# Mahdi-Si/VAE-TEB

Measured on AMD Instinct MI355X. Metric: train samples/sec + ELBO, 4096-pt windows, batch 256, 1/2/4/8 MI355X, higher is better.
Workload: dtype bf16 MFMA (decoder heads + conv blocks + ResidualMLP linears, LSTM recurrences f16 fwd / bf16 bwd), fp32 accumulation; fp32 LayerNorm / BatchNorm / LSTM state / front-end / optimizer

## Files before the change

include/vaeteb.h:

```cpp
#ifndef VAETEB_H
#define VAETEB_H

#include <stdint.h>

#ifdef __cplusplus
extern "C" {
#endif

#define VT_OK 0
#define VT_ERR_ARG (-1)
#define VT_ERR_LAYOUT (-2)
#define VT_ERR_HIP (-3)

#define VT_FFT_MAX_LDS 8192

const char* vt_last_error(void);
int vt_stream_fork(void* from, void* to);
int vt_stream_mark(void* stream, int* slot);
int vt_stream_wait_mark(void* stream, int slot);
int vt_abi_version(void);
int vt_arrive_reset(void* stream);
int vt_capture_info(void* stream, char* buf, int len);
int vt_set_h16_format(int fp16);
int vt_get_h16_format(void);


int vt_fe_spectrum(const float* x, int64_t rows, int N, int n_pad, int pad_left, int pad_mode, const void* tw,
                   void* xhat, void* stream);
int vt_fe_spectrum_rolled(const float* x, int64_t B, int64_t x_row_stride, int N, int n_pad, int pad_left,
                          int pad_mode, const int* shifts, int K, const void* tw, void* xhat, void* stream);

int vt_fe_lowpass(const float* x, int64_t rows, int64_t x_row_stride, int N, int n_pad, int pad_left,
                  const float* h0, int radius, int step, int start, int S, float* out, int64_t out_row_stride,
                  void* stream);

int vt_fe_wavelet(const void* xhat, int64_t B, int C, int n_pad, const float* psi, int n_items, const int* items,
                  const void* tw, int N, int pad_left, void* analytic, int n_slots, const float* h0, int radius,
                  int step, int start, int S, float* s1, int s1_channels, void* stream);

int vt_fe_pairs(const void* analytic, int64_t B, int n_slots, int N, int n_pad, int pad_left, int n_pairs,
                const int* slot_i, const int* slot_j, const float* power, const void* tw, const float* phi0, int dec,
                int start, int S, int pad_mode, float* out, void* stream);
int vt_fe_pairs_split(const void* analytic_i, int n_slots_i, const void* analytic_j, int n_slots_j, int64_t B, int K,
                      int N, int n_pad, int pad_left, int n_pairs, const int* slot_i, const int* slot_j,
                      const float* power, const void* tw, const float* phi0, int dec, int start, int S,
                      int pad_mode, float* out, void* stream);

int vt_fe_set_pairs_persist(int grid);
int vt_fe_set_pairs_direct(int on);
int vt_fe_set_pairs_half(int on);
int vt_fe_set_analytic_polar(int on);

int vt_fe_set_pairs_stamps(void* buf);

int vt_fe_normalize(const float* in, int64_t B, int C, int in_C, int S, const int* kind, const float* mean, const float* stdv,
                    float log_eps, float* out, int out_C, int out_off, void* stream);
int vt_fe_normalize_window(const float* in, int64_t B, int C, int in_C, int in_S, int s0, int S_len,
// ... 348 lines not shown
```

vae-teb_amd/csrc/abi.cpp:

```cpp
#include <stdarg.h>
#include <stdio.h>
#include <stdlib.h>

#include <atomic>
#include <utility>
#include <vector>

#include "common.h"

namespace vt {
static thread_local char g_err[512] = "";

void set_error(const char* fmt, ...) {
    va_list ap;
    va_start(ap, fmt);
    vsnprintf(g_err, sizeof(g_err), fmt, ap);
    va_end(ap);
}

unsigned arrive_slots(unsigned n, hipStream_t st) {
    static std::atomic<unsigned> next[2];
    constexpr unsigned HALF = ARRIVE_POOL / 2;
    hipStreamCaptureStatus cs = hipStreamCaptureStatusNone;
    const int cap = (st && hipStreamIsCapturing(st, &cs) == hipSuccess && cs == hipStreamCaptureStatusActive) ? 1 : 0;
    for (;;) {
        const unsigned b = next[cap].fetch_add(n) % HALF;
        if (b + n <= HALF) return b + cap * HALF;
    }
}

static std::vector<std::pair<const void*, size_t>>& arrive_pools() {
    static std::vector<std::pair<const void*, size_t>> v;
    return v;
}
int register_arrive_pool(const void* sym, size_t bytes) {
    arrive_pools().emplace_back(sym, bytes);
    return (int)arrive_pools().size();
}

static std::atomic<int> g_h16{0};
int h16_format() { return g_h16.load(std::memory_order_relaxed); }
}

extern "C" {
const char* vt_last_error(void) { return vt::g_err; }

int vt_arrive_reset(void* stream) {
    for (const auto& [sym, bytes] : vt::arrive_pools()) {
        void* p = nullptr;
        if (hipGetSymbolAddress(&p, sym) != hipSuccess || hipMemsetAsync(p, 0, bytes, vt::S(stream)) != hipSuccess) {
            vt::set_error("vt_arrive_reset: cannot clear a counter pool");
            return VT_ERR_HIP;
        }
    }
    return VT_OK;
}
int vt_abi_version(void) { return 1; }
int vt_set_h16_format(int fp16) { return vt::g_h16.exchange(fp16 ? 1 : 0); }
int vt_get_h16_format(void) { return vt::h16_format(); }
}

namespace {
constexpr int kForkEvents = 1024, kMaxDevices = 16;
hipEvent_t g_fork_ev[kMaxDevices][kForkEvents];
std::atomic<unsigned> g_fork_next[kMaxDevices];

struct SlotRec {
    unsigned long long cap;
    void* stream;
};
SlotRec g_slot[kMaxDevices][kForkEvents];
int g_trace = -1;

unsigned long long capture_id(void* stream, bool* capturing) {
    hipStreamCaptureStatus st = hipStreamCaptureStatusNone;
    unsigned long long id = 0;
    if (hipStreamGetCaptureInfo((hipStream_t)stream, &st, &id) != hipSuccess) {
        (void)hipGetLastError();
        st = hipStreamCaptureStatusNone;
    }
    *capturing = st == hipStreamCaptureStatusActive;
    return *capturing ? id : 0ull;
}

bool trace() {
    if (g_trace < 0) {
        const char* e = getenv("VAETEB_EVENT_TRACE");
        g_trace = e && e[0] == '1';
    }
    return g_trace;
}
}
// ... 118 lines not shown
```

vae-teb_amd/csrc/common.h:

```cpp
#pragma once
#include <hip/hip_runtime.h>
#include <stdint.h>

#include "../../include/vaeteb.h"

namespace vt {

void set_error(const char* fmt, ...);
const void* bucket_marker_kernel();

#define VT_CHECK_ARG(cond, ...)                  \
    do {                                         \
        if (!(cond)) {                           \
            ::vt::set_error(__VA_ARGS__);        \
            return VT_ERR_ARG;                   \
        }                                        \
    } while (0)

#define VT_LAUNCH_CHECK(name)                                                     \
    do {                                                                          \
        hipError_t e_ = hipGetLastError();                                        \
        if (e_ != hipSuccess) {                                                   \
            ::vt::set_error("%s: %s", name, hipGetErrorString(e_));               \
            return VT_ERR_HIP;                                                    \
// ... 40 lines not shown
}

__device__ __forceinline__ bool last_arrival(unsigned* ctr, unsigned total) {
    __shared__ unsigned s_last;
    asm volatile("s_waitcnt vmcnt(0)" ::: "memory");
    __syncthreads();
    if (threadIdx.x == 0) {
        const unsigned old = atomicAdd(ctr, 1u);
        const bool last = old == total - 1;
        if (last) atomicExch(ctr, 0u);
        s_last = last ? 1u : 0u;
    }
    __syncthreads();
    return s_last != 0u;
}

__device__ __forceinline__ float wave_sum(float v) {
#pragma unroll
    for (int o = 32; o > 0; o >>= 1) v += __shfl_xor(v, o, 64);
    return v;
}

__device__ __forceinline__ float block_sum(float v, float* red) {
    v = wave_sum(v);
    const int lane = threadIdx.x & 63, w = threadIdx.x >> 6, nw = (blockDim.x + 63) >> 6;
    __syncthreads();
    if (lane == 0) red[w] = v;
    __syncthreads();
    float t = 0.f;
    for (int i = 0; i < nw; ++i) t += red[i];
    return t;
}

__device__ __forceinline__ int reflect_idx(int i, int n) {
    if (n == 1) return 0;
    const int p = 2 * (n - 1);
    i %= p;
    if (i < 0) i += p;
    return i < n ? i : p - i;
}

__device__ __forceinline__ int pad_src(int i, int n, int mode) {
    if (mode == 0) return reflect_idx(i, n);
    if (mode == 1) return (i < 0 || i >= n) ? -1 : i;
    i %= n;
    return i < 0 ? i + n : i;
}

}
```

vae-teb_amd/csrc/gemm.hip:

```cpp
#include <algorithm>

#include "common.h"
#include "skinny.h"

namespace vt {

static constexpr int TM = 64, TN = 64, TK = 16, GT = 256;

struct RowMajor {
    const float* p;
    int64_t ld;
    __device__ float at(int64_t r, int64_t c) const { return p[r * ld + c]; }
};
struct ColMajor {
    const float* p;
    int64_t ld;
    __device__ float at(int64_t r, int64_t c) const { return p[c * ld + r]; }
};

struct ConvGeom {
    int B, L_in, Cin, Cout, K;
    int up;
    int mode;
    int L_up;
// ... 176 lines not shown
            for (; r + 3 * rpi < r1; r += 4 * rpi) {
                a0 += X[r * N + c];
                a1 += X[(r + rpi) * N + c];
                a2 += X[(r + 2 * rpi) * N + c];
                a3 += X[(r + 3 * rpi) * N + c];
            }
            for (; r < r1; r += rpi) a0 += X[r * N + c];
        }
        const float a = (a0 + a1) + (a2 + a3);
        red[threadIdx.x] = a;
        __syncthreads();
        if (threadIdx.x < N) {
            float s = 0.f;
            for (int i = 0; i < rpi; ++i) s += red[i * N + threadIdx.x];
            partial[(int64_t)blockIdx.x * N + threadIdx.x] = s;
        }
    } else {
        const int n = blockIdx.y * 256 + threadIdx.x;
        if (n >= N) return;
        float a = 0.f;
        for (int64_t r = r0; r < r1; ++r) a += X[r * N + n];
        partial[(int64_t)blockIdx.x * N + n] = a;
    }
}
__global__ __launch_bounds__(256) void k_colsum_final(const float* __restrict__ partial, int blocks, int N,
                                                      float* __restrict__ out, int accumulate) {
    __shared__ float red[16];
    const int n = blockIdx.x;
    float a = 0.f;
#pragma unroll 8
    for (int b = threadIdx.x; b < blocks; b += 256) a += partial[(int64_t)b * N + n];
    a = block_sum(a, red);
    if (threadIdx.x == 0) out[n] = accumulate ? out[n] + a : a;
}

template <bool UP>
__global__ void k_conv_fold(const float* __restrict__ gpad, ConvGeom g, float rcin, float* __restrict__ dx,
                            int accumulate) {
    const int i = blockIdx.x * blockDim.x + threadIdx.x;
    if (i >= g.L_in * g.Cin) return;
    const int b = blockIdx.y;
    const int Lp = g.L_out + g.K - 1;
    const float* gb0 = gpad + (int64_t)b * Lp * g.Cin;
    float out;
    if (!UP && g.mode == 0) {
        out = gb0[g.pad * g.Cin + i];
    } else {
        int s = rcin != 0.f ? (int)((float)i * rcin) : i / g.Cin;
        if (s * g.Cin > i) --s;
        else if ((s + 1) * g.Cin <= i) ++s;
        const int ci = i - s * g.Cin;
        const float* gb = gb0 + ci;
        auto gup = [&](int t) -> float {
            float v = gb[(t + g.pad) * g.Cin];
            if (g.mode == 0) return v;
            if (g.L_up <= g.pad) {
                if (t == 0)
                    for (int tp = 0; tp < g.pad; ++tp) v += gb[tp * g.Cin];
                if (t == g.L_up - 1)
                    for (int tp = g.pad + g.L_up; tp < Lp; ++tp) v += gb[tp * g.Cin];
                return v;
            }
            if (t >= 1 && t <= g.pad) v += gb[(g.pad - t) * g.Cin];
            const int tr = g.pad + 2 * (g.L_up - 1) - t;
            if (t <= g.L_up - 2 && tr < Lp && tr >= g.pad + g.L_up) v += gb[tr * g.Cin];
            return v;
// ... 127 lines not shown
                                                  K, nullptr, accumulate, ws, ws_floats, vt_gemm_splits_hint(N, K, R),
                                                  0, 0, 0, S(stream));
}

int vt_conv1d_fold(const float* gpad, int B, int L_in, int Cin, int Cout, int K, int mode, int up, float* dX,
                   int accumulate, void* stream) {
    VT_CHECK_ARG(B > 0 && L_in > 0 && Cin > 0, "vt_conv1d_fold: shape");
    ConvGeom g = make_geom(B, L_in, Cin, Cout, K, mode, up);
    const int rc = fold_launch(gpad, g, dX, accumulate, S(stream));
    if (rc) return rc;
    VT_LAUNCH_CHECK("vt_conv1d_fold");
    return VT_OK;
}

int vt_linear_ln_fwd(const float* X, int64_t R, int K, const float* W, int N, const float* bias, const float* gamma,
                     const float* beta, int act, float eps, float* Y, float* xhat, float* rstd, void* stream) {
    VT_CHECK_ARG(R > 0 && K > 0 && N > 0 && N <= SK_MAX_N && gamma && beta && act >= 0 && act <= 3,
                 "vt_linear_ln_fwd: shape (N <= %d)", SK_MAX_N);
    sk_linear_ln_fwd(X, R, K, W, N, bias, gamma, beta, act, eps, Y, xhat, rstd, S(stream));
    VT_LAUNCH_CHECK("vt_linear_ln_fwd");
    return VT_OK;
}

int vt_colsum(const float* X, int64_t R, int N, float* out, int accumulate, float* ws, int64_t ws_floats,
              void* stream) {
    VT_CHECK_ARG(R > 0 && N > 0, "vt_colsum: shape");
    const int64_t rows = N <= 256 ? 64 : 8;
    int64_t blocks = (R + rows - 1) / rows;
    if (blocks > 1024) blocks = 1024;
    if (blocks * N > ws_floats) blocks = ws_floats / N;
    VT_CHECK_ARG(blocks >= 1, "vt_colsum: workspace too small");
    const int64_t rpb = (R + blocks - 1) / blocks;
    blocks = (R + rpb - 1) / rpb;
    hipLaunchKernelGGL(k_colsum_partial, dim3((unsigned)blocks, N <= 256 ? 1 : (unsigned)((N + 255) / 256)),
                       dim3(256), 0, S(stream), X, R, N, rpb, ws);
    hipLaunchKernelGGL(k_colsum_final, dim3(N), dim3(256), 0, S(stream), ws, (int)blocks, N, out,
                       accumulate);
    VT_LAUNCH_CHECK("vt_colsum");
    return VT_OK;
}

int vt_conv1d_out_len(int L_in, int K, int mode, int up) { return make_geom(1, L_in, 1, 1, K, mode, up).L_out; }

int vt_conv1d_fwd(const float* X, int B, int L_in, int Cin, const float* W, int Cout, int K, int mode, int up,
                  float* Y, void* stream) {
    VT_CHECK_ARG(B > 0 && L_in > 0 && Cin > 0 && Cout > 0 && K > 0 && (mode == 0 || mode == 1),
                 "vt_conv1d_fwd: shape");
    ConvGeom g = make_geom(B, L_in, Cin, Cout, K, mode, up);
    VT_CHECK_ARG(mode == 0 || g.L_up > 1, "vt_conv1d_fwd: length");
    const int64_t M = (int64_t)B * g.L_out;
    return launch<Im2col, ConvW, false, false>("vt_conv1d_fwd", Im2col{X, g}, ConvW{W, Cin, K}, M, Cout,
                                               (int64_t)K * Cin, Y, Cout, nullptr, 0, nullptr, 0, 1, 0, 0, 0,
                                               S(stream));
}

int vt_conv1d_bwd_data(const float* dY, int B, int L_in, int Cin, const float* W, int Cout, int K, int mode, int up,
                       float* dX, int accumulate, float* gpad, void* stream) {
    VT_CHECK_ARG(B > 0 && L_in > 0 && Cin > 0 && Cout > 0 && K > 0, "vt_conv1d_bwd_data: shape");
    ConvGeom g = make_geom(B, L_in, Cin, Cout, K, mode, up);
    const int Lp = g.L_out + K - 1;
    const int64_t M = (int64_t)B * Lp;
    int rc = launch<Col2imA, ConvWT, false, false>("vt_conv1d_bwd_data", Col2imA{dY, g.L_out, Lp, Cout},
                                                   ConvWT{W, Cin, Cout, K}, M, Cin, (int64_t)K * Cout, gpad, Cin,
                                                   nullptr, 0, nullptr, 0, 1, 0, 0, 0, S(stream));
    if (rc) return rc;
    rc = fold_launch(gpad, g, dX, accumulate, S(stream));
// ... 19 lines not shown
```

vae-teb_amd/csrc/mfma.hip:

```cpp
#include "h16.h"

namespace vt {

constexpr int QM = 256, QN = 64, QK = 64, QT = 512;
constexpr int ROWB = QK * 2;
constexpr int A_BYTES = QM * ROWB;
constexpr int B_BYTES = QN * ROWB;
constexpr int NA = 3, NB = 8;
constexpr int GEMM_LDS = NA * A_BYTES + NB * B_BYTES;

__device__ __forceinline__ int swz(int r, int c) { return c ^ ((r >> 1) & 7); }

__device__ __forceinline__ void glds16(const void* src, char* lds) {
    __builtin_amdgcn_global_load_lds((const __attribute__((address_space(1))) void*)src,
                                     (__attribute__((address_space(3))) void*)lds, 16, 0, 0);
}

VT_ARRIVE_POOL(g_arrive_gemm);

typedef unsigned u32x4 __attribute__((ext_vector_type(4)));
__device__ __forceinline__ void st_agent4(__amdgpu_buffer_rsrc_t r, unsigned off, f32x4 v) {
    __builtin_amdgcn_raw_buffer_store_b128(__builtin_bit_cast(u32x4, v), r, (int)off, 0, CPOL_SC1);
}
__device__ __forceinline__ f32x4 ld_agent4(__amdgpu_buffer_rsrc_t r, unsigned off) {
// ... 106 lines not shown
                s += p == z ? acc[g >> 2][g & 3] : ld_agent4(pr, (unsigned)(p * slab + (g * QT + tid) * 16));
            acc[g >> 2][g & 3] = s;
        }
    }
#pragma unroll
    for (int i = 0; i < 2; ++i)
#pragma unroll
        for (int j = 0; j < 4; ++j) {
            const int col = n0 + 16 * j + lr;
            const float bcol = bias ? bias[col] : 0.f;
#pragma unroll
            for (int r = 0; r < 4; ++r) {
                const int row = m0 + 32 * w + 16 * i + 4 * lc + r;
                if (row >= M) continue;
                float o = acc[i][j][r] + bcol;
                if (accumulate) o = C[(int64_t)row * ldc + col] + o;
                C[(int64_t)row * ldc + col] = o;
            }
        }
}

template <typename H>
__global__ void k_bf16_rows(const float* __restrict__ X, int64_t M, int K, H* __restrict__ out, int64_t Mpad,
                            int Kpad) {
    const int64_t i = (int64_t)blockIdx.x * blockDim.x + threadIdx.x;
    const int64_t total = Mpad * Kpad;
    if (i >= total) return;
    const int64_t m = i / Kpad;
    const int k = (int)(i - m * Kpad);
    out[i] = (m < M && k < K) ? (H)X[m * K + k] : (H)0.f;
}

template <typename H>
__global__ __launch_bounds__(256) void k_bf16_transpose(const float* __restrict__ X, int64_t R, int Cn,
                                                        H* __restrict__ out, int64_t Cpad, int64_t Rpad) {
    __shared__ float tile[64][65];
    const int64_t r0 = (int64_t)blockIdx.x * 64, c0 = (int64_t)blockIdx.y * 64;
    const int tx = threadIdx.x & 63, ty = threadIdx.x >> 6;
    for (int i = ty; i < 64; i += 4) {
        const int64_t r = r0 + i, c = c0 + tx;
        tile[i][tx] = (r < R && c < Cn) ? X[r * Cn + c] : 0.f;
    }
    __syncthreads();
    for (int i = ty; i < 64; i += 4) {
        const int64_t c = c0 + i, r = r0 + tx;
        if (c < Cpad && r < Rpad) out[c * Rpad + r] = (H)tile[tx][i];
    }
}

template <typename H>
__global__ __launch_bounds__(256) void k_bf16_shadow(const float* __restrict__ W, int N, int K,
                                                     H* __restrict__ W16, H* __restrict__ W16t) {
    __shared__ float tile[64][65];
    const int64_t n0 = (int64_t)blockIdx.y * 64, k0 = (int64_t)blockIdx.x * 64;
    const int tx = threadIdx.x & 63, ty = threadIdx.x >> 6;
    for (int i = ty; i < 64; i += 4) {
        const float v = W[(n0 + i) * K + k0 + tx];
        tile[i][tx] = v;
        W16[(n0 + i) * K + k0 + tx] = (H)v;
    }
    __syncthreads();
    for (int i = ty; i < 64; i += 4) W16t[(k0 + i) * N + n0 + tx] = (H)tile[tx][i];
}

typedef short v4i16 __attribute__((ext_vector_type(4)));
typedef short v8i16 __attribute__((ext_vector_type(8)));
// ... 136 lines not shown

}

using namespace vt;

extern "C" {

int vt_mfma_supported(int K, int N) { return (K > 0 && N > 0 && K % QK == 0 && N % QN == 0) ? 1 : 0; }

int vt_mfma_workspace_floats(int64_t R, int K, int N, int64_t* floats) {
    VT_CHECK_ARG(R > 0 && K > 0 && N > 0 && floats, "vt_mfma_workspace_floats: shape");
    MfmaPlan f = plan(R, N, K), d = plan(R, K, N), w = plan(N, K, R);
    const int64_t wf = w.a_floats + up_to((int64_t)K * w.Kpad / 2, 64) + w.part_floats + N;
    int64_t m = f.a_floats + f.part_floats;
    if (d.a_floats + d.part_floats > m) m = d.a_floats + d.part_floats;
    if (wf > m) m = wf;
    *floats = m;
    return VT_OK;
}

int vt_mfma_weight_shadow(const float* W, int N, int K, void* W16, void* W16t, void* stream) {
    VT_CHECK_ARG(vt_mfma_supported(K, N) && W && W16 && W16t, "vt_mfma_weight_shadow: K and N must be multiples of 64");
    VT_H16(hipLaunchKernelGGL(k_bf16_shadow<H>, dim3(K / 64, N / 64), dim3(256), 0, S(stream), W, N, K, (H*)W16,
                              (H*)W16t));
    VT_LAUNCH_CHECK("vt_mfma_weight_shadow");
    return VT_OK;
}

int vt_mfma_linear_fwd(const float* X, int64_t R, int K, const void* W16, int N, const float* bias, float* Y,
                       float* ws, int64_t ws_floats, void* stream) {
    VT_CHECK_ARG(R > 0 && vt_mfma_supported(K, N), "vt_mfma_linear_fwd: K and N must be positive multiples of 64");
    MfmaPlan p = plan(R, N, K);
    VT_CHECK_ARG(p.a_floats + p.part_floats <= ws_floats, "vt_mfma_linear_fwd: workspace too small");
    const int64_t tot = p.Mpad * p.Kpad;
    int rc = VT_OK;
    VT_H16(H* A = (H*)ws;
           hipLaunchKernelGGL(k_bf16_rows<H>, dim3((unsigned)((tot + 255) / 256)), dim3(256), 0, S(stream), X, R, K, A,
                              p.Mpad, (int)p.Kpad);
           rc = run("vt_mfma_linear_fwd", (const H*)A, (const H*)W16, K, R, N, p, Y, bias, 0, ws + p.a_floats,
                    S(stream)));
    return rc;
}

int vt_mfma_linear_bwd_data(const float* dY, int64_t R, int N, const void* W16t, int K, float* dX, int accumulate,
                            float* ws, int64_t ws_floats, void* stream) {
    VT_CHECK_ARG(R > 0 && vt_mfma_supported(N, K), "vt_mfma_linear_bwd_data: K and N must be positive multiples of 64");
    MfmaPlan p = plan(R, K, N);
    VT_CHECK_ARG(p.a_floats + p.part_floats <= ws_floats, "vt_mfma_linear_bwd_data: workspace too small");
    const int64_t tot = p.Mpad * p.Kpad;
    int rc = VT_OK;
    VT_H16(H* A = (H*)ws;
           hipLaunchKernelGGL(k_bf16_rows<H>, dim3((unsigned)((tot + 255) / 256)), dim3(256), 0, S(stream), dY, R, N, A,
                              p.Mpad, (int)p.Kpad);
           rc = run("vt_mfma_linear_bwd_data", (const H*)A, (const H*)W16t, N, R, K, p, dX, nullptr, accumulate,
                    ws + p.a_floats, S(stream)));
    return rc;
}

int vt_mfma_linear_bwd_weight(const float* dY, int64_t R, int N, const float* X, int K, float* dW, float* db,
                              int accumulate, float* ws, int64_t ws_floats, void* stream) {
    VT_CHECK_ARG(R > 0 && vt_mfma_supported(K, N), "vt_mfma_linear_bwd_weight: K and N must be positive multiples of 64");
    if (N % DWT == 0 && K % DWT == 0) {
        VT_H16(hipLaunchKernelGGL(k_mfma_dw<H>, dim3(K / DWT, N / DWT), dim3(256), 0, S(stream), dY, R, N, X, K, dW,
                                  accumulate));
        VT_LAUNCH_CHECK("vt_mfma_linear_bwd_weight");
        return db ? vt_colsum(dY, R, N, db, accumulate, ws, ws_floats, stream) : VT_OK;
    }
    MfmaPlan p = plan(N, K, R);
    const int64_t b_floats = up_to((int64_t)K * p.Kpad / 2, 64);
    VT_CHECK_ARG(p.a_floats + b_floats + p.part_floats + N <= ws_floats, "vt_mfma_linear_bwd_weight: workspace too small");
    float* part = ws + p.a_floats + b_floats;
    int rc = VT_OK;
    VT_H16(H* A = (H*)ws;
           H* Bt = (H*)(ws + p.a_floats);
           hipLaunchKernelGGL(k_bf16_transpose<H>, dim3((unsigned)(p.Kpad / 64), (unsigned)(p.Mpad / 64)), dim3(256), 0,
                              S(stream), dY, R, N, A, p.Mpad, p.Kpad);
           hipLaunchKernelGGL(k_bf16_transpose<H>, dim3((unsigned)(p.Kpad / 64), (unsigned)(K / 64)), dim3(256), 0,
                              S(stream), X, R, K, Bt, (int64_t)K, p.Kpad);
           rc = run("vt_mfma_linear_bwd_weight", (const H*)A, (const H*)Bt, p.Kpad, N, K, p, dW, nullptr, accumulate,
                    part, S(stream)));
    if (rc || !db) return rc;
    return vt_colsum(dY, R, N, db, accumulate, part, ws_floats - p.a_floats - b_floats, stream);
}

}
```

vae-teb_amd/csrc/norm.hip:

```cpp
#include <math.h>
#include <stdlib.h>

#include "bnbwd.h"
#include "common.h"
#include "dropout.h"

namespace vt {

enum Act { ACT_NONE = 0, ACT_RELU = 1, ACT_GELU = 2, ACT_TANH = 3 };

__device__ __forceinline__ float act_f(float z, int act) {
    switch (act) {
        case ACT_RELU: return z > 0.f ? z : 0.f;
        case ACT_GELU: return 0.5f * z * (1.f + erff(z * 0.70710678118654752f));
        case ACT_TANH: return tanhf(z);
        default: return z;
    }
}
__device__ __forceinline__ float act_d(float z, int act) {
    switch (act) {
        case ACT_RELU: return z > 0.f ? 1.f : 0.f;
        case ACT_GELU: {
            const float cdf = 0.5f * (1.f + erff(z * 0.70710678118654752f));
            const float pdf = 0.39894228040143268f * expf(-0.5f * z * z);
// ... 139 lines not shown
            b += red[i][1][c];
        }
        part[(int64_t)blockIdx.x * 2 * C + c] = a;
        part[(int64_t)blockIdx.x * 2 * C + C + c] = b;
    }
}

__global__ __launch_bounds__(NT) void k_ln_bwd_wide(const float* __restrict__ dy, const float* __restrict__ xhat,
                                                    const float* __restrict__ rstd, int C,
                                                    const float* __restrict__ gamma, const float* __restrict__ beta,
                                                    int act, float* __restrict__ dx, float* __restrict__ rowpart) {
    __shared__ float red[16];
    const int64_t row = blockIdx.x;
    const float* dyr = dy + row * C;
    const float* hr = xhat + row * C;
    float s1 = 0.f, s2 = 0.f;
    for (int c = threadIdx.x; c < C; c += NT) {
        const float h = hr[c];
        const float dz = dyr[c] * act_d(h * gamma[c] + beta[c], act);
        const float g = dz * gamma[c];
        s1 += g;
        s2 += g * h;
        rowpart[row * 2 * C + c] = dz * h;
        rowpart[row * 2 * C + C + c] = dz;
    }
    const float m1 = block_sum(s1, red) / (float)C;
    const float m2 = block_sum(s2, red) / (float)C;
    const float rs = rstd[row];
    for (int c = threadIdx.x; c < C; c += NT) {
        const float h = hr[c];
        const float dz = dyr[c] * act_d(h * gamma[c] + beta[c], act);
        dx[row * C + c] = rs * (dz * gamma[c] - m1 - h * m2);
    }
}

template <int CTRL>
__device__ __forceinline__ float dppf(float v) {
    return __builtin_bit_cast(float, __builtin_amdgcn_update_dpp(0, __builtin_bit_cast(int, v), CTRL, 0xF, 0xF, false));
}
__device__ __forceinline__ float sum16(float v) {
    v += dppf<0xB1>(v);
    v += dppf<0x4E>(v);
    const float r4 = dppf<0x124>(v), r12 = dppf<0x12C>(v);
    v += (threadIdx.x & 4) ? r4 : r12;
    v += dppf<0x128>(v);
    return v;
}

template <int CPL>
__global__ __launch_bounds__(NT) void k_ln_fwd16(const float* __restrict__ x, int64_t R, int C,
                                                 const float* __restrict__ gamma, const float* __restrict__ beta,
                                                 int act, float eps, float* __restrict__ y, float* __restrict__ xhat,
                                                 float* __restrict__ rstd_out) {
    const int lr = threadIdx.x & 15;
    const int64_t row = (int64_t)blockIdx.x * (NT / 16) + (threadIdx.x >> 4);
    const bool ok = row < R;
    const float* xr = x + (ok ? row : 0) * C;
    float v[CPL], s = 0.f;
#pragma unroll
    for (int j = 0; j < CPL; ++j) {
        const int c = lr + 16 * j;
        v[j] = (ok && c < C) ? xr[c] : 0.f;
        s += v[j];
    }
    const float mean = sum16(s) / (float)C;
    float q = 0.f;
// ... 809 lines not shown
                     float* ws, int64_t ws_floats, void* stream) {
    VT_CHECK_ARG(R > 0 && C > 0, "vt_layernorm_bwd: shape");
    hipStream_t st = S(stream);
    if (C <= 256) {
        int64_t blocks = (R + 63) / 64;
        if (blocks > 1024) blocks = 1024;
        if (blocks * 2 * C > ws_floats) blocks = ws_floats / (2 * C);
        VT_CHECK_ARG(blocks >= 1, "vt_layernorm_bwd: workspace too small");
        const int64_t rpb = (R + blocks - 1) / blocks;
        blocks = (R + rpb - 1) / rpb;
        const dim3 grid((unsigned)blocks);
#define VT_LNB(CPL) hipLaunchKernelGGL(k_ln_bwd16<CPL>, grid, dim3(NT), 0, st, dy, xhat, rstd, R, C, gamma, beta, act, \
                                       rpb, dx, ws)
        if (C <= 32) VT_LNB(2);
        else if (C <= 64) VT_LNB(4);
        else if (C <= 128) VT_LNB(8);
        else VT_LNB(16);
#undef VT_LNB
        hipLaunchKernelGGL(k_colred16, dim3((unsigned)((2 * C + CR_C - 1) / CR_C)), dim3(NT), 0, st, ws, (int)blocks,
                           2 * C, dgamma, dbeta, C, accumulate_params);
    } else if (C <= 512) {
        int64_t blocks = (R + 63) / 64;
        if (blocks > 1024) blocks = 1024;
        if (blocks * 2 * C > ws_floats) blocks = ws_floats / (2 * C);
        VT_CHECK_ARG(blocks >= 1, "vt_layernorm_bwd: workspace too small");
        const int64_t rpb = (R + blocks - 1) / blocks;
        blocks = (R + rpb - 1) / rpb;
        hipLaunchKernelGGL(k_ln_bwd<8>, dim3((unsigned)blocks), dim3(NT), 0, st, dy, xhat, rstd, R, C, gamma, beta,
                           act, rpb, dx, ws);
        hipLaunchKernelGGL(k_reduce_parts, dim3(2 * C), dim3(NT), 0, st, ws, (int)blocks, 2 * C, dgamma,
                           dbeta, C, accumulate_params);
    } else {
        VT_CHECK_ARG(ws_floats >= 2 * R * C, "vt_layernorm_bwd: workspace too small (wide)");
        hipLaunchKernelGGL(k_ln_bwd_wide, dim3((unsigned)R), dim3(NT), 0, st, dy, xhat, rstd, C, gamma, beta, act, dx,
                           ws);
        hipLaunchKernelGGL(k_reduce_parts, dim3(2 * C), dim3(NT), 0, st, ws, (int)R, 2 * C, dgamma, dbeta,
                           C, accumulate_params);
    }
    VT_LAUNCH_CHECK("vt_layernorm_bwd");
    return VT_OK;
}

static int bn_blocks(int64_t M, int64_t ws_floats, int C, int64_t* rpb) {
    auto need = [&](int64_t b) { return ((2 * C * b + 1) & ~(int64_t)1) + 4 * C * ((b + BN_GB - 1) / BN_GB); };
    int64_t blocks = (M + 255) / 256;
    const int64_t cap = C <= 128 && g_bn_fold ? BN_FOLD_BLOCKS : 2048;
    if (blocks > cap) blocks = cap;
    while (blocks > 1 && need(blocks) > ws_floats) blocks = blocks * 15 / 16 < blocks - 1 ? blocks * 15 / 16 : blocks - 1;
    if (need(blocks) > ws_floats) return 0;
    *rpb = ((M + blocks - 1) / blocks + 3) / 4 * 4;
    return (int)((M + *rpb - 1) / *rpb);
}

static BnFin fin_of(int mode, int64_t M) {
    BnFin f{};
    f.mode = mode;
    f.M = M;
    return f;
}

int vt_batchnorm_fwd(const float* x, int64_t M, int C, const float* gamma, const float* beta, int act, float eps,
                     float momentum, float* y, float* mean, float* rstd, float* run_mean, float* run_var, float* ws,
                     int64_t ws_floats, void* stream) {
    VT_CHECK_ARG(M > 0 && C > 0 && C <= 256, "vt_batchnorm_fwd: shape (C <= 256)");
    int64_t rpb;
    const int blocks = bn_blocks(M, ws_floats, C, &rpb);
    VT_CHECK_ARG(blocks >= 1, "vt_batchnorm_fwd: workspace too small");
    hipStream_t st = S(stream);
    BnFin f0 = fin_of(0, M);
    f0.mean = mean;
// ... 200 lines not shown
```

vae-teb_amd/vaeteb/_lib.py:

```python
import ctypes
import os
import re

import torch

_HERE = os.path.dirname(os.path.abspath(__file__))
_ROOT = os.path.dirname(os.path.dirname(_HERE))
LIB_PATH = os.environ.get("VAETEB_LIB", os.path.join(_HERE, "_lib", "libvaeteb.so"))
HEADER = os.path.join(_ROOT, "include", "vaeteb.h")

VT_ERR_ARG, VT_ERR_LAYOUT, VT_ERR_HIP = -1, -2, -3

_CT = {
    "int": ctypes.c_int, "int64_t": ctypes.c_int64, "float": ctypes.c_float, "double": ctypes.c_double,
    "void*": ctypes.c_void_p, "float*": ctypes.c_void_p, "double*": ctypes.c_void_p, "int*": ctypes.c_void_p, "int32_t*": ctypes.c_void_p, "int64_t*": ctypes.c_void_p,
    "char*": ctypes.c_char_p,
}


def parse_header(path=HEADER):
    src = open(path).read()
    src = re.sub(r"/\*.*?\*/", " ", src, flags=re.S)
    protos = {}
    for m in re.finditer(r"\b(const\s+char\s*\*|int|void)\s+(vt_\w+)\s*\(([^)]*)\)\s*;", src):
# ... 70 lines not shown


def stream():
    return torch._C._cuda_getCurrentRawStream(torch._C._cuda_getDevice())


def call(name, *args):
    return lib().call(name, *args)


def wait_for(waiter, src=None):
    w = waiter if isinstance(waiter, int) else waiter.cuda_stream
    s = stream() if src is None else (src if isinstance(src, int) else src.cuda_stream)
    if w != s:
        rc = lib().fns["vt_stream_fork"](s, w)
        if rc != 0:
            raise RuntimeError(f"vt_stream_fork: {lib().last_error()}")


_H16 = [None]


def set_h16(fp16):
    v = 1 if fp16 else 0
    if _H16[0] != v:
        lib().fns["vt_set_h16_format"](v)
        _H16[0] = v


def h16():
    return "fp16" if lib().fns["vt_get_h16_format"]() else "bf16"


def capture_info(src=None):
    import ctypes
    buf = ctypes.create_string_buffer(1 << 16)
    s = stream() if src is None else (src if isinstance(src, int) else src.cuda_stream)
    call("vt_capture_info", s, buf, len(buf))
    return buf.value.decode()


def mark(src=None):
    import ctypes
    slot = ctypes.c_int()
    call("vt_stream_mark", stream() if src is None else src.cuda_stream, ctypes.byref(slot))
    return slot.value


def wait_mark(slot, waiter=None):
    call("vt_stream_wait_mark", stream() if waiter is None else waiter.cuda_stream, slot)
```

Baseline: 34070.

## Fuse wide LayerNorm backward and column sums into single-pass kernels; vectorize bf16 row packing

```diff
diff --git a/include/vaeteb.h b/include/vaeteb.h
--- a/include/vaeteb.h
+++ b/include/vaeteb.h
@@ -23,6 +23,7 @@
 int vt_capture_info(void* stream, char* buf, int len);
 int vt_set_h16_format(int fp16);
 int vt_get_h16_format(void);
+int vt_set_wide_glue_legacy(int on);
 
 
 int vt_fe_spectrum(const float* x, int64_t rows, int N, int n_pad, int pad_left, int pad_mode, const void* tw,
diff --git a/vae-teb_amd/csrc/abi.cpp b/vae-teb_amd/csrc/abi.cpp
--- a/vae-teb_amd/csrc/abi.cpp
+++ b/vae-teb_amd/csrc/abi.cpp
@@ -40,6 +40,9 @@
 
 static std::atomic<int> g_h16{0};
 int h16_format() { return g_h16.load(std::memory_order_relaxed); }
+
+static std::atomic<int> g_wide_legacy{getenv("VAETEB_WIDE_GLUE_LEGACY") ? atoi(getenv("VAETEB_WIDE_GLUE_LEGACY")) != 0 : 0};
+int wide_glue_legacy() { return g_wide_legacy.load(std::memory_order_relaxed); }
 }
 
 extern "C" {
@@ -58,6 +61,7 @@
 int vt_abi_version(void) { return 1; }
 int vt_set_h16_format(int fp16) { return vt::g_h16.exchange(fp16 ? 1 : 0); }
 int vt_get_h16_format(void) { return vt::h16_format(); }
+int vt_set_wide_glue_legacy(int on) { return vt::g_wide_legacy.exchange(on ? 1 : 0); }
 }
 
 namespace {
diff --git a/vae-teb_amd/csrc/common.h b/vae-teb_amd/csrc/common.h
--- a/vae-teb_amd/csrc/common.h
+++ b/vae-teb_amd/csrc/common.h
@@ -96,6 +96,32 @@
     return t;
 }
 
+constexpr int CT_C = 16;
+__device__ __forceinline__ void ct_wave_sums(float (&a)[CT_C], float (*red)[CT_C]) {
+    const int lane = threadIdx.x & 63, w = threadIdx.x >> 6;
+#pragma unroll
+    for (int o = 32; o > 0; o >>= 1) {
+        float t[CT_C];
+#pragma unroll
+        for (int j = 0; j < CT_C; ++j) t[j] = __shfl_xor(a[j], o, 64);
+#pragma unroll
+        for (int j = 0; j < CT_C; ++j) a[j] += t[j];
+    }
+    if (lane == 0) {
+#pragma unroll
+        for (int j = 0; j < CT_C; ++j) red[w][j] = a[j];
+    }
+    __syncthreads();
+}
+__device__ __forceinline__ float ct_total(const float (*red)[CT_C], int j) {
+    float t = 0.f;
+#pragma unroll
+    for (int i = 0; i < 4; ++i) t += red[i][j];
+    return t;
+}
+
+int wide_glue_legacy();
+
 __device__ __forceinline__ int reflect_idx(int i, int n) {
     if (n == 1) return 0;
     const int p = 2 * (n - 1);
diff --git a/vae-teb_amd/csrc/gemm.hip b/vae-teb_amd/csrc/gemm.hip
--- a/vae-teb_amd/csrc/gemm.hip
+++ b/vae-teb_amd/csrc/gemm.hip
@@ -232,6 +232,55 @@
     for (int b = threadIdx.x; b < blocks; b += 256) a += partial[(int64_t)b * N + n];
     a = block_sum(a, red);
     if (threadIdx.x == 0) out[n] = accumulate ? out[n] + a : a;
+}
+
+__global__ __launch_bounds__(256) void k_colsum_wide(const float* __restrict__ X, int64_t M, int N,
+                                                     int64_t rows_per_block, int blocks, float* __restrict__ out,
+                                                     int accumulate) {
+    static_assert(CT_C == 16, "16 columns x 16 partial groups");
+    __shared__ float sp[256][CT_C + 1];
+    __shared__ float red[4][CT_C];
+    const int tid = threadIdx.x, cc = tid & (CT_C - 1), q = tid >> 4;
+    const int c0 = blockIdx.x * CT_C, c = c0 + cc;
+    float acc[CT_C];
+#pragma unroll
+    for (int j = 0; j < CT_C; ++j) acc[j] = 0.f;
+    for (int b0 = 0; b0 < blocks; b0 += 256) {
+        for (int i = 0; i < 16; i += 2) {
+            const int ba = b0 + q + 16 * i, bb = ba + 16;
+            if (ba >= blocks) break;
+            const int64_t r0a = (int64_t)ba * rows_per_block, r0b = (int64_t)bb * rows_per_block;
+            const int64_t r1a = c >= N ? r0a : (r0a + rows_per_block < M ? r0a + rows_per_block : M);
+            const int64_t r1b = c >= N || bb >= blocks ? r0b : (r0b + rows_per_block < M ? r0b + rows_per_block : M);
+            float pa = 0.f, pb = 0.f;
+            for (int64_t k = 0; k < rows_per_block; k += 8) {
+                float va[8], vb[8];
+#pragma unroll
+                for (int u = 0; u < 8; ++u) {
+                    va[u] = r0a + k + u < r1a ? X[(r0a + k + u) * N + c] : 0.f;
+                    vb[u] = r0b + k + u < r1b ? X[(r0b + k + u) * N + c] : 0.f;
+                }
+#pragma unroll
+                for (int u = 0; u < 8; ++u) {
+                    if (r0a + k + u < r1a) pa += va[u];
+                    if (r0b + k + u < r1b) pb += vb[u];
+                }
+            }
+            sp[q + 16 * i][cc] = pa;
+            if (bb < blocks) sp[q + 16 * i + 16][cc] = pb;
+        }
+        __syncthreads();
+        if (b0 + tid < blocks) {
+#pragma unroll
+            for (int j = 0; j < CT_C; ++j) acc[j] += sp[tid][j];
+        }
+        __syncthreads();
+    }
+    ct_wave_sums(acc, red);
+    if (tid < CT_C && c0 + tid < N) {
+        const float v = ct_total(red, tid);
+        out[c0 + tid] = accumulate ? out[c0 + tid] + v : v;
+    }
 }
 
 template <bool UP>
@@ -425,6 +474,12 @@
     VT_CHECK_ARG(blocks >= 1, "vt_colsum: workspace too small");
     const int64_t rpb = (R + blocks - 1) / blocks;
     blocks = (R + rpb - 1) / rpb;
+    if (N > 256 && R <= 16384 && !wide_glue_legacy()) {
+        hipLaunchKernelGGL(k_colsum_wide, dim3((unsigned)((N + CT_C - 1) / CT_C)), dim3(256), 0, S(stream), X, R, N, rpb,
+                           (int)blocks, out, accumulate);
+        VT_LAUNCH_CHECK("vt_colsum");
+        return VT_OK;
+    }
     hipLaunchKernelGGL(k_colsum_partial, dim3((unsigned)blocks, N <= 256 ? 1 : (unsigned)((N + 255) / 256)),
                        dim3(256), 0, S(stream), X, R, N, rpb, ws);
     hipLaunchKernelGGL(k_colsum_final, dim3(N), dim3(256), 0, S(stream), ws, (int)blocks, N, out,
diff --git a/vae-teb_amd/csrc/mfma.hip b/vae-teb_amd/csrc/mfma.hip
--- a/vae-teb_amd/csrc/mfma.hip
+++ b/vae-teb_amd/csrc/mfma.hip
@@ -162,6 +162,33 @@
 }
 
 template <typename H>
+__global__ __launch_bounds__(256) void k_bf16_rows4(const float4* __restrict__ X, int64_t M, int K4,
+                                                    hv4<H>* __restrict__ out, int64_t Mpad, int Kpad4) {
+    const int k4 = blockIdx.x * 64 + (threadIdx.x & 63);
+    if (k4 >= Kpad4) return;
+    for (int64_t m = (int64_t)blockIdx.y * 4 + (threadIdx.x >> 6); m < Mpad; m += 4 * (int64_t)gridDim.y) {
+        hv4<H> o = {(H)0.f, (H)0.f, (H)0.f, (H)0.f};
+        if (m < M && k4 < K4) {
+            const float4 v = X[m * K4 + k4];
+            o = hv4<H>{(H)v.x, (H)v.y, (H)v.z, (H)v.w};
+        }
+        out[m * Kpad4 + k4] = o;
+    }
+}
+
+template <typename H>
+static void launch_rows(const float* X, int64_t M, int K, H* out, int64_t Mpad, int Kpad, hipStream_t st) {
+    if (K % 4 == 0 && Kpad % 4 == 0 && (uintptr_t)X % 16 == 0 && (uintptr_t)out % 8 == 0 && !wide_glue_legacy()) {
+        const int64_t gy = (Mpad + 3) / 4;
+        hipLaunchKernelGGL(k_bf16_rows4<H>, dim3((unsigned)((Kpad / 4 + 63) / 64), (unsigned)(gy < 65535 ? gy : 65535)),
+                           dim3(256), 0, st, (const float4*)X, M, K / 4, (hv4<H>*)out, Mpad, Kpad / 4);
+        return;
+    }
+    const int64_t tot = Mpad * Kpad;
+    hipLaunchKernelGGL(k_bf16_rows<H>, dim3((unsigned)((tot + 255) / 256)), dim3(256), 0, st, X, M, K, out, Mpad, Kpad);
+}
+
+template <typename H>
 __global__ __launch_bounds__(256) void k_bf16_transpose(const float* __restrict__ X, int64_t R, int Cn,
                                                         H* __restrict__ out, int64_t Cpad, int64_t Rpad) {
     __shared__ float tile[64][65];
@@ -364,11 +391,9 @@
     VT_CHECK_ARG(R > 0 && vt_mfma_supported(K, N), "vt_mfma_linear_fwd: K and N must be positive multiples of 64");
     MfmaPlan p = plan(R, N, K);
     VT_CHECK_ARG(p.a_floats + p.part_floats <= ws_floats, "vt_mfma_linear_fwd: workspace too small");
-    const int64_t tot = p.Mpad * p.Kpad;
     int rc = VT_OK;
     VT_H16(H* A = (H*)ws;
-           hipLaunchKernelGGL(k_bf16_rows<H>, dim3((unsigned)((tot + 255) / 256)), dim3(256), 0, S(stream), X, R, K, A,
-                              p.Mpad, (int)p.Kpad);
+           launch_rows<H>(X, R, K, A, p.Mpad, (int)p.Kpad, S(stream));
            rc = run("vt_mfma_linear_fwd", (const H*)A, (const H*)W16, K, R, N, p, Y, bias, 0, ws + p.a_floats,
                     S(stream)));
     return rc;
@@ -379,11 +404,9 @@
     VT_CHECK_ARG(R > 0 && vt_mfma_supported(N, K), "vt_mfma_linear_bwd_data: K and N must be positive multiples of 64");
     MfmaPlan p = plan(R, K, N);
     VT_CHECK_ARG(p.a_floats + p.part_floats <= ws_floats, "vt_mfma_linear_bwd_data: workspace too small");
-    const int64_t tot = p.Mpad * p.Kpad;
     int rc = VT_OK;
     VT_H16(H* A = (H*)ws;
-           hipLaunchKernelGGL(k_bf16_rows<H>, dim3((unsigned)((tot + 255) / 256)), dim3(256), 0, S(stream), dY, R, N, A,
-                              p.Mpad, (int)p.Kpad);
+           launch_rows<H>(dY, R, N, A, p.Mpad, (int)p.Kpad, S(stream));
            rc = run("vt_mfma_linear_bwd_data", (const H*)A, (const H*)W16t, N, R, K, p, dX, nullptr, accumulate,
                     ws + p.a_floats, S(stream)));
     return rc;
diff --git a/vae-teb_amd/csrc/norm.hip b/vae-teb_amd/csrc/norm.hip
--- a/vae-teb_amd/csrc/norm.hip
+++ b/vae-teb_amd/csrc/norm.hip
@@ -195,6 +195,152 @@
         const float dz = dyr[c] * act_d(h * gamma[c] + beta[c], act);
         dx[row * C + c] = rs * (dz * gamma[c] - m1 - h * m2);
     }
+}
+
+__device__ __forceinline__ float ln_dz(float dy, float h, float gm, float bt, int act) {
+#pragma clang fp contract(off)
+    return dy * act_d(fmaf(h, gm, bt), act);
+}
+
+__device__ __forceinline__ void block_sum2(float& a, float& b, float (*red)[NT / 64]) {
+#pragma unroll
+    for (int o = 32; o > 0; o >>= 1) {
+        const float ta = __shfl_xor(a, o, 64), tb = __shfl_xor(b, o, 64);
+        a += ta;
+        b += tb;
+    }
+    const int lane = threadIdx.x & 63, w = threadIdx.x >> 6;
+    __syncthreads();
+    if (lane == 0) {
+        red[0][w] = a;
+        red[1][w] = b;
+    }
+    __syncthreads();
+    float ta = 0.f, tb = 0.f;
+#pragma unroll
+    for (int i = 0; i < NT / 64; ++i) {
+        ta += red[0][i];
+        tb += red[1][i];
+    }
+    a = ta;
+    b = tb;
+}
+
+template <int V>
+__device__ __forceinline__ void ln_bwd_wide_row(const float* __restrict__ dy, const float* __restrict__ xhat,
+                                                const float* __restrict__ rstd, int64_t row, int C,
+                                                const float* __restrict__ gamma, const float* __restrict__ beta,
+                                                int act, float* __restrict__ dx) {
+#pragma clang fp contract(off)
+    __shared__ float red[2][NT / 64];
+    const float* dyr = dy + row * C;
+    const float* hr = xhat + row * C;
+    float* dxr = dx + row * C;
+    float s1 = 0.f, s2 = 0.f;
+    if constexpr (V > 0) {
+        float dv[V], hv[V], gm[V], bt[V];
+#pragma unroll
+        for (int j = 0; j < V; ++j) {
+            const int c = threadIdx.x + NT * j;
+            const bool ok = c < C;
+            dv[j] = ok ? dyr[c] : 0.f;
+            hv[j] = ok ? hr[c] : 0.f;
+            gm[j] = ok ? gamma[c] : 0.f;
+            bt[j] = ok ? beta[c] : 0.f;
+        }
+#pragma unroll
+        for (int j = 0; j < V; ++j) {
+            if (threadIdx.x + NT * j >= C) continue;
+            dv[j] = ln_dz(dv[j], hv[j], gm[j], bt[j], act) * gm[j];
+            s1 = s1 + dv[j];
+            s2 = s2 + dv[j] * hv[j];
+        }
+        block_sum2(s1, s2, red);
+        const float m1 = s1 / (float)C, m2 = s2 / (float)C;
+        const float rs = rstd[row];
+#pragma unroll
+        for (int j = 0; j < V; ++j) {
+            const int c = threadIdx.x + NT * j;
+            if (c < C) dxr[c] = rs * ((dv[j] - m1) - hv[j] * m2);
+        }
+    } else {
+        for (int c = threadIdx.x; c < C; c += NT) {
+            const float h = hr[c];
+            const float g = ln_dz(dyr[c], h, gamma[c], beta[c], act) * gamma[c];
+            s1 = s1 + g;
+            s2 = s2 + g * h;
+        }
+        block_sum2(s1, s2, red);
+        const float m1 = s1 / (float)C, m2 = s2 / (float)C;
+        const float rs = rstd[row];
+        for (int c = threadIdx.x; c < C; c += NT) {
+            const float h = hr[c];
+            const float g = ln_dz(dyr[c], h, gamma[c], beta[c], act) * gamma[c];
+            dxr[c] = rs * ((g - m1) - h * m2);
+        }
+    }
+}
+
+__device__ __forceinline__ void ln_bwd_wide_cols(const float* __restrict__ dy, const float* __restrict__ xhat,
+                                                 int64_t R, int C, int tile, const float* __restrict__ gamma,
+                                                 const float* __restrict__ beta, int act,
+                                                 float* __restrict__ dgamma, float* __restrict__ dbeta,
+                                                 int accumulate) {
+#pragma clang fp contract(off)
+    static_assert(NT == 256 && CT_C == 16, "16 columns x 16 row groups, 4 waves");
+    __shared__ float sg[NT][CT_C + 1], sb[NT][CT_C + 1];
+    __shared__ float red[2][4][CT_C];
+    const int tid = threadIdx.x, cc = tid & (CT_C - 1), q = tid >> 4;
+    const int c0 = tile * CT_C, c = c0 + cc;
+    const bool okc = c < C;
+    const float gm = okc ? gamma[c] : 0.f, bt = okc ? beta[c] : 0.f;
+    float ag[CT_C], ab[CT_C];
+#pragma unroll
+    for (int j = 0; j < CT_C; ++j) ag[j] = ab[j] = 0.f;
+    for (int64_t r0 = 0; r0 < R; r0 += NT) {
+        float dv[16], hv[16];
+#pragma unroll
+        for (int i = 0; i < 16; ++i) {
+            const int64_t r = r0 + q + 16 * i;
+            const bool ok = okc && r < R;
+            dv[i] = ok ? dy[r * C + c] : 0.f;
+            hv[i] = ok ? xhat[r * C + c] : 0.f;
+        }
+#pragma unroll
+        for (int i = 0; i < 16; ++i) {
+            const float dz = ln_dz(dv[i], hv[i], gm, bt, act);
+            sg[q + 16 * i][cc] = dz * hv[i];
+            sb[q + 16 * i][cc] = dz;
+        }
+        __syncthreads();
+        if (r0 + tid < R) {
+#pragma unroll
+            for (int j = 0; j < CT_C; ++j) {
+                ag[j] = ag[j] + sg[tid][j];
+                ab[j] = ab[j] + sb[tid][j];
+            }
+        }
+        __syncthreads();
+    }
+    ct_wave_sums(ag, red[0]);
+    ct_wave_sums(ab, red[1]);
+    if (tid < 2 * CT_C && c0 + cc < C) {
+        const float v = ct_total(red[q], cc);
+        float* o = (q ? dbeta : dgamma) + c0 + cc;
+        *o = accumulate ? *o + v : v;
+    }
+}
+
+template <int V>
+__global__ __launch_bounds__(NT) void k_ln_bwd_wide2(const float* __restrict__ dy, const float* __restrict__ xhat,
+                                                     const float* __restrict__ rstd, int64_t R, int C,
+                                                     const float* __restrict__ gamma, const float* __restrict__ beta,
+                                                     int act, float* __restrict__ dx, float* __restrict__ dgamma,
+                                                     float* __restrict__ dbeta, int accumulate) {
+    if (blockIdx.x < R)
+        ln_bwd_wide_row<V>(dy, xhat, rstd, (int64_t)blockIdx.x, C, gamma, beta, act, dx);
+    else
+        ln_bwd_wide_cols(dy, xhat, R, C, (int)(blockIdx.x - R), gamma, beta, act, dgamma, dbeta, accumulate);
 }
 
 template <int CTRL>
@@ -1070,10 +1216,22 @@
                            dbeta, C, accumulate_params);
     } else {
         VT_CHECK_ARG(ws_floats >= 2 * R * C, "vt_layernorm_bwd: workspace too small (wide)");
-        hipLaunchKernelGGL(k_ln_bwd_wide, dim3((unsigned)R), dim3(NT), 0, st, dy, xhat, rstd, C, gamma, beta, act, dx,
-                           ws);
-        hipLaunchKernelGGL(k_reduce_parts, dim3(2 * C), dim3(NT), 0, st, ws, (int)R, 2 * C, dgamma, dbeta,
-                           C, accumulate_params);
+        if (wide_glue_legacy()) {
+            hipLaunchKernelGGL(k_ln_bwd_wide, dim3((unsigned)R), dim3(NT), 0, st, dy, xhat, rstd, C, gamma, beta, act,
+                               dx, ws);
+            hipLaunchKernelGGL(k_reduce_parts, dim3(2 * C), dim3(NT), 0, st, ws, (int)R, 2 * C, dgamma, dbeta,
+                               C, accumulate_params);
+        } else {
+#define VT_LNR(V) hipLaunchKernelGGL(k_ln_bwd_wide2<V>, dim3((unsigned)(R + tiles)), dim3(NT), 0, st, dy, xhat, rstd, R, C, \
+                                     gamma, beta, act, dx, dgamma, dbeta, accumulate_params)
+            const int64_t tiles = (C + CT_C - 1) / CT_C;
+            VT_CHECK_ARG(R + tiles <= 0x7fffffff, "vt_layernorm_bwd: too many rows");
+            if (C <= 4 * NT) VT_LNR(4);
+            else if (C <= 8 * NT) VT_LNR(8);
+            else if (C <= 16 * NT) VT_LNR(16);
+            else VT_LNR(0);
+#undef VT_LNR
+        }
     }
     VT_LAUNCH_CHECK("vt_layernorm_bwd");
     return VT_OK;
diff --git a/vae-teb_amd/vaeteb/_lib.py b/vae-teb_amd/vaeteb/_lib.py
--- a/vae-teb_amd/vaeteb/_lib.py
+++ b/vae-teb_amd/vaeteb/_lib.py
@@ -126,6 +126,10 @@
     return "fp16" if lib().fns["vt_get_h16_format"]() else "bf16"
 
 
+def set_wide_glue_legacy(on):
+    return bool(lib().fns["vt_set_wide_glue_legacy"](1 if on else 0))
+
+
 def capture_info(src=None):
     import ctypes
     buf = ctypes.create_string_buffer(1 << 16)
```

New measurement: 34270, median of 6. No clear change (+0.6%).
